# bcosm/MonteCarloOptionsPricer

Measured on AMD Instinct MI355X. Metric: Mpaths/sec at 252 steps, higher is better.
Workload: dtype f64; 1 GPU; C2: European call, GBM, 10M paths x 252 steps per GPU, fp64 matrix written; collective=none, seed=20251031

## Files before the change

### include/mcgpu_debug.h

```cpp
#ifndef MCGPU_DEBUG_H
#define MCGPU_DEBUG_H
#include "mcgpu.h"
#ifdef __cplusplus
extern "C" {
#endif

int mcg_debug_eval(mcg_ctx* ctx, int fn, const double* x, double* y, int64_t n);
int mcg_debug_lsm_hooks(mcg_ctx* ctx, long long spin_limit, int poll_delay);
int mcg_debug_lsm_date_fault(mcg_ctx* ctx, int mode, int date, int workgroup, int delay, long long spin_limit);
int mcg_debug_batch_budget(mcg_ctx* ctx, size_t bytes);
int mcg_debug_coalesce_slots(int max_slots);
int mcg_debug_coalesce_selftest(int n_threads, int calls_per_thread, int* wrong);
int mcg_debug_peer_decision(int same_process, int bus_id_resolves, int same_device, int can_access_peer);
int mcg_debug_shm_attach(const char* name, int n_ranks, int rank, double timeout_s, void** handle);
int mcg_debug_shm_barrier(void* handle);
int mcg_debug_shm_poison(void* handle);
int mcg_debug_shm_detach(void* handle);

#ifdef __cplusplus
}
#endif
#endif
```

### montecarlooptionspricer_amd/_native.py

```python
from __future__ import annotations

import ctypes as C
import os
import sys

_HERE = os.path.dirname(os.path.abspath(__file__))
_LIB = os.environ.get("MCG_LIB") or os.path.join(_HERE, "lib", "libmcgpu.so")

MCG_OK = 0
K_GBM, K_RBERGOMI, K_PAYOFF, K_LSM_SWEEP, K_LSM_SOLVE, K_TRANSPOSE, K_ASYM, K_MARTINGALE, K_BRANCHING, K_BATCH = range(10)
KERNEL_NAMES = {K_GBM: "gbm", K_RBERGOMI: "rbergomi", K_PAYOFF: "payoff", K_LSM_SWEEP: "lsm_sweep",
                K_LSM_SOLVE: "lsm_solve", K_TRANSPOSE: "transpose", K_ASYM: "asymptotic", K_MARTINGALE: "martingale", K_BRANCHING: "branching", K_BATCH: "batch_rows"}

ALLREDUCE_FN = C.CFUNCTYPE(C.c_int, C.c_void_p, C.c_void_p, C.c_int, C.c_void_p)


class Row(C.Structure):
    _fields_ = [("S0", C.c_double), ("xi", C.c_double), ("H", C.c_double), ("eta", C.c_double), ("rho", C.c_double),
                ("strike", C.c_double), ("maturity", C.c_double), ("sigma", C.c_double), ("dividend", C.c_double),
                ("n_steps", C.c_int), ("is_call", C.c_int)]


class Stats(C.Structure):
    _fields_ = [(k, C.c_int64) for k in (
# ... 36 lines not shown
    vp = C.c_void_p
    L.mcg_last_error.restype = C.c_char_p
    L.mcg_version.restype = C.c_char_p
    L.mcg_device_count.argtypes = [C.POINTER(C.c_int)]
    L.mcg_init.argtypes = [C.POINTER(vp), C.c_int]
    L.mcg_init_on_stream.argtypes = [C.POINTER(vp), C.c_int, vp]
    L.mcg_finalize.argtypes = [vp]
    L.mcg_synchronize.argtypes = [vp]
    L.mcg_trim.argtypes = [vp]
    L.mcg_set_allreduce.argtypes = [vp, ALLREDUCE_FN, vp]
    L.mcg_comm_unique_id.argtypes = [C.c_char_p]
    L.mcg_comm_init_rank.argtypes = [vp, C.c_char_p, C.c_int, C.c_int]
    L.mcg_comm_init_shm.argtypes = [vp, C.c_char_p, C.c_int, C.c_int]

    def newer(name, argtypes):
        try:
            getattr(L, name).argtypes = argtypes
        except AttributeError:
            if not os.environ.get("MCG_LIB"):
                raise

    newer("mcg_comm_shm_peer_mailbox", [vp, C.c_int, C.POINTER(C.c_int)])
    newer("mcg_debug_shm_attach", [C.c_char_p, C.c_int, C.c_int, C.c_double, C.POINTER(vp)])
    newer("mcg_debug_shm_barrier", [vp])
    newer("mcg_debug_shm_poison", [vp])
    newer("mcg_debug_shm_detach", [vp])
    newer("mcg_lsm_one_launch_reset", [vp])
    newer("mcg_debug_lsm_hooks", [vp, C.c_longlong, C.c_int])
    newer("mcg_comm_info", [vp] + [C.POINTER(C.c_int)] * 4)
    newer("mcg_timing_select", [vp, C.c_uint])
    newer("mcg_stats", [C.POINTER(Stats), C.c_int])
    newer("mcg_debug_lsm_date_fault", [vp, C.c_int, C.c_int, C.c_int, C.c_int, C.c_longlong])
    newer("mcg_debug_batch_budget", [vp, C.c_size_t])
    newer("mcg_debug_peer_decision", [C.c_int] * 4)
    newer("mcg_probe_write_ceiling", [vp, C.c_int64, C.c_int, C.c_int, C.POINTER(C.c_double), C.POINTER(C.c_double)])
    newer("mcg_generator_clock_arm", [vp, C.c_int])
    newer("mcg_generator_clock", [vp, C.POINTER(C.c_double), C.POINTER(C.c_int), C.POINTER(C.c_double), C.POINTER(C.c_double)])
    newer("mcg_row_features", [C.POINTER(C.c_double), C.c_size_t, C.POINTER(C.c_double), C.POINTER(C.c_double)])
    newer("mcg_row_build", [C.POINTER(C.c_double), C.c_size_t, C.c_double, C.c_double, C.c_double, C.c_int, C.c_double,
                            C.POINTER(Row), C.POINTER(C.c_double)])
    newer("mcg_batch_price_rows6", [vp, C.POINTER(Row), C.POINTER(C.c_double), C.c_int64, C.c_int, C.c_double, C.c_double, C.c_int,
                                    C.c_int, C.c_int, C.c_uint64, C.POINTER(C.c_double)])
    L.mcg_paths_gbm.argtypes = [vp, C.c_uint64, C.c_double, C.c_double, C.c_double, C.c_double, C.c_int,
                                C.c_uint64, C.c_int64, C.POINTER(vp)]
    L.mcg_paths_gbm_payoff.argtypes = [vp, C.c_uint64, C.c_double, C.c_double, C.c_double, C.c_double, C.c_int,
                                       C.c_uint64, C.c_int64, C.c_double, C.c_int, C.POINTER(vp)]
    L.mcg_paths_rbergomi.argtypes = [vp, C.c_uint64] + [C.c_double] * 7 + [C.c_int, C.c_uint64, C.c_int64,
                                                                          C.POINTER(vp)]
    L.mcg_paths_rbergomi_payoff.argtypes = [vp, C.c_uint64] + [C.c_double] * 7 + [C.c_int, C.c_uint64, C.c_int64,
                                                                                 C.c_double, C.c_int, C.POINTER(vp)]
    L.mcg_paths_from_host.argtypes = [vp, dp, C.c_int64, C.c_int, C.POINTER(vp)]
    L.mcg_paths_to_host.argtypes = [vp, dp]
    L.mcg_paths_to_host_step_major.argtypes = [vp, dp]
    L.mcg_paths_info.argtypes = [vp, C.POINTER(C.c_int64), C.POINTER(C.c_int), C.POINTER(C.c_int64), C.POINTER(vp)]
    L.mcg_paths_free.argtypes = [vp]
    L.mcg_price_european.argtypes = [vp, vp, C.c_double, C.c_double, C.c_double, C.c_int, dp, dp]
    L.mcg_price_lsm.argtypes = [vp, vp, C.c_double, C.c_double, C.c_double, C.c_double, C.c_int, C.c_int, dp, dp]
    L.mcg_lsm_one_launch_enabled.argtypes = [vp, C.POINTER(C.c_int)]
    L.mcg_price_asymptotic.argtypes = [vp, vp] + [C.c_double] * 4 + [C.c_int, C.c_double, C.c_double, dp]
    L.mcg_compat_asymptotic_price.argtypes = [dp, C.c_int64, C.c_int] + [C.c_double] * 4 + [C.c_int, C.c_double, C.c_double, dp]
    L.mcg_price_martingale.argtypes = [vp, vp] + [C.c_double] * 4 + [C.c_int, C.c_int, C.c_int, dp, dp, dp]
    L.mcg_compat_martingale_price.argtypes = [dp, C.c_int64, C.c_int] + [C.c_double] * 4 + [C.c_int, C.c_int, C.c_int, dp]
    ip = C.POINTER(C.c_int)
    L.mcg_price_branching.argtypes = [vp, vp] + [C.c_double] * 4 + [C.c_int, C.c_int, ip, C.c_int, C.c_uint64, dp, dp, dp]
    L.mcg_compat_branching_price.argtypes = [dp, C.c_int64, C.c_int] + [C.c_double] * 4 + [C.c_int, C.c_int, ip, C.c_int, dp]
    L.mcg_batch_price_rows.argtypes = [vp, C.POINTER(Row), C.c_int64, C.c_int, C.c_double, C.c_double, C.c_int, C.c_int,
# ... 23 lines not shown
```

### montecarlooptionspricer_amd/csrc/kernels_gbm.hip

```cpp
#include <algorithm>
#include <cstdlib>
#include <vector>

#include "devmath.hpp"
#include "fastmath.hpp"
#include "mcg_internal.hpp"

#ifndef MCG_GBM_TABLES
#define MCG_GBM_TABLES 0
#endif

namespace mcg {

struct GbmArgs {
    double* out;
    int64_t ld;
    int64_t n_paths;
    int n_steps;
    uint64_t path_begin;
    uint32_t k0, k1;
    double S0, drift, vol;
    fm::LogScale ls;
    double K;
    int is_call;
    double* partials;
    const double2* log_tab;
    unsigned long long* clk;
    unsigned clk_first, clk_shift;
};

template <bool PAYOFF, int MODE, int PPL>
__global__ __launch_bounds__(256) void k_gbm_paths(GbmArgs a) {
    constexpr bool SMALL = MODE >= 1;
    typedef double v2d __attribute__((ext_vector_type(2)));
#if MCG_GBM_TABLES == 0
    typedef fm::Tables GbmTables;
    __shared__ GbmTables tabs;
    if (MODE >= 2) fm::load_tables_scaled(&tabs, a.log_tab, a.vol * a.vol);
    else fm::load_tables(&tabs, a.log_tab);
#else
    typedef fm::NormalTables<MCG_GBM_TABLES == 1 ? 10 : 9> GbmTables;
    __shared__ GbmTables tabs;
    fm::load_normal_tables(&tabs, a.log_tab, MODE >= 2 ? a.vol * a.vol : 1.0);
#endif
    const GbmTables* tab = &tabs;
    __syncthreads();
#ifdef MCG_GBM_NO_STAMPS
    const bool stamps = false;
#else
    const bool stamps = a.clk != nullptr && (blockIdx.x & ((1u << a.clk_shift) - 1u)) == a.clk_first;
#endif
    __shared__ unsigned long long stamp0[3];
    if (threadIdx.x == 0) {
        stamp0[2] = 0;
        if (stamps && (blockIdx.x >> a.clk_shift) < (unsigned)GBM_CLK_SLOTS) {
            stamp0[2] = (unsigned long long)(a.clk + 2 * (blockIdx.x >> a.clk_shift));
            stamp0[0] = __builtin_amdgcn_s_memtime();
            stamp0[1] = __builtin_amdgcn_s_memrealtime();
        }
    }
    const int64_t i = ((int64_t)blockIdx.x * 256 + threadIdx.x) * PPL;
    const bool in_row = PPL == 1 || i < a.ld;
    double S[PPL];
#pragma unroll
    for (int p = 0; p < PPL; ++p) S[p] = a.S0;
    if (in_row) {
        double* row = a.out + (int64_t)blockIdx.x * (256 * PPL);
        const unsigned lane_bytes = threadIdx.x * (8u * PPL);
        auto store_row = [&](double* r) {
            if constexpr (PPL == 1) {
                asm volatile("global_store_dwordx2 %0, %1, %2 nt" : : "v"(lane_bytes), "v"(S[0]), "s"(r) : "memory");
            } else {
                const v2d v = {S[0], S[PPL - 1]};
                asm volatile("global_store_dwordx4 %0, %1, %2 nt\n\ts_nop 1" : : "v"(lane_bytes), "v"(v), "s"(r) : "memory");
            }
        };
        store_row(row);
        PhiloxLane lane_rng[PPL];
#pragma unroll
        for (int p = 0; p < PPL; ++p) lane_rng[p] = philox_lane_setup(a.path_begin + (uint64_t)(i + p), STREAM_PRICE, a.k1);
        auto step = [&](const double (&e)[PPL]) {
#pragma unroll
            for (int p = 0; p < PPL; ++p)
                S[p] = MODE == 3 ? fm::scaled_exp_small6(S[p], e[p]) : SMALL ? fm::scaled_exp_small(S[p], e[p]) : fm::scaled_exp(S[p], e[p]);
            row += a.ld;
            store_row(row);
        };
        auto pair_exponents = [&](uint32_t wa, uint32_t wb, double& e0, double& e1) {
            if (MODE >= 2) fm::box_muller_pair_affine_scaled(wa, wb, tab, a.ls, a.drift, e0, e1);
            else fm::box_muller_pair_affine(wa, wb, tab, a.vol, a.drift, e0, e1);
        };
        const int n_blocks = a.n_steps >> 2;
#pragma unroll 1
        for (int b = 0; b < n_blocks; ++b) {
            Philox4 w[PPL];
#pragma unroll
            for (int p = 0; p < PPL; ++p) w[p] = philox4x32_10_lane(lane_rng[p], (uint32_t)b, a.k0, a.k1);
            double e0[PPL], e1[PPL];
#pragma unroll
            for (int p = 0; p < PPL; ++p) pair_exponents(w[p].w0, w[p].w1, e0[p], e1[p]);
            step(e0);
            step(e1);
#pragma unroll
            for (int p = 0; p < PPL; ++p) pair_exponents(w[p].w2, w[p].w3, e0[p], e1[p]);
            step(e0);
            step(e1);
        }
        const int rest = a.n_steps & 3;
        if (rest) {
            Philox4 w[PPL];
#pragma unroll
            for (int p = 0; p < PPL; ++p) w[p] = philox4x32_10_lane(lane_rng[p], (uint32_t)n_blocks, a.k0, a.k1);
            double e0[PPL], e1[PPL];
#pragma unroll
            for (int p = 0; p < PPL; ++p) pair_exponents(w[p].w0, w[p].w1, e0[p], e1[p]);
            step(e0);
            if (rest >= 2) step(e1);
            if (rest == 3) {
#pragma unroll
                for (int p = 0; p < PPL; ++p) pair_exponents(w[p].w2, w[p].w3, e0[p], e1[p]);
                step(e0);
            }
        }
    }
    if (threadIdx.x == 0 && stamp0[2] != 0) {
        const unsigned long long c1 = __builtin_amdgcn_s_memtime(), r1 = __builtin_amdgcn_s_memrealtime();
        unsigned long long* dst = (unsigned long long*)stamp0[2];
        dst[0] = c1 - stamp0[0];
        dst[1] = r1 - stamp0[1];
    }
    if (PAYOFF) {
        __shared__ double red[2 * 4];
        double v[2] = {0.0, 0.0};
#pragma unroll
        for (int p = 0; p < PPL; ++p) {
            const double pay = (in_row && i + p < a.n_paths) ? payoff_of(a.is_call != 0, S[p], a.K) : 0.0;
            v[0] += pay;
            v[1] += pay * pay;
        }
        block_sum<2, 4>(v, red);
        if (threadIdx.x == 0) {
            a.partials[2 * (int64_t)blockIdx.x] = v[0];
            a.partials[2 * (int64_t)blockIdx.x + 1] = v[1];
        }
    }
}

__global__ __launch_bounds__(256) void k_payoff_sums(const double* last_row, int64_t n_paths, double K,
                                                     int is_call, double* partials) {
    __shared__ double red[2 * 4];
    double v[2] = {0.0, 0.0};
    for (int64_t i = (int64_t)blockIdx.x * 256 + threadIdx.x; i < n_paths; i += (int64_t)gridDim.x * 256) {
        const double pay = payoff_of(is_call != 0, last_row[i], K);
        v[0] += pay;
        v[1] += pay * pay;
    }
    block_sum<2, 4>(v, red);
    if (threadIdx.x == 0) {
        partials[2 * (int64_t)blockIdx.x] = v[0];
        partials[2 * (int64_t)blockIdx.x + 1] = v[1];
    }
}

constexpr int64_t FIN_CHUNK = 8192;

__device__ __forceinline__ void sum_pairs(const double* partials, int64_t n, double (&v)[2], double* red) {
    v[0] = 0.0;
    v[1] = 0.0;
    for (int64_t b = threadIdx.x; b < n; b += 1024) {
        v[0] += partials[2 * b];
        v[1] += partials[2 * b + 1];
// ... 35 lines not shown
        TimedLaunch t(ctx, MCG_K_PAYOFF);
        hipLaunchKernelGGL(k_sum_chunks, dim3((unsigned)n_chunks), dim3(1024), 0, ctx->stream, src, n, ctx->fin_chunks);
        src = ctx->fin_chunks;
        n = n_chunks;
    }
    {
        TimedLaunch t(ctx, MCG_K_PAYOFF);
        hipLaunchKernelGGL(k_finish_sums, dim3(1), dim3(1024), 0, ctx->stream, src, n, (double)n_local, d);
    }
    MCG_HIP(hipGetLastError());
    if (ctx->allreduce) {
        if (ctx->allreduce(ctx->allreduce_user, d, 3, (void*)ctx->stream) != 0)
            return fail(MCG_ERR_COMM, "all-reduce of payoff sums failed");
    }
    MCG_HIP(hipMemcpyAsync(ctx->h_scalars + SC_SUMS, d, 3 * sizeof(double), hipMemcpyDeviceToHost, ctx->stream));
    MCG_HIP(hipStreamSynchronize(ctx->stream));
    out3[0] = ctx->h_scalars[SC_SUMS];
    out3[1] = ctx->h_scalars[SC_SUMS + 1];
    out3[2] = ctx->h_scalars[SC_SUMS + 2];
    return MCG_OK;
}

template <bool PAYOFF, int PPL>
static void launch_gbm_mode(mcg_ctx* ctx, const GbmArgs& a, int mode, unsigned n_blocks) {
    const dim3 grid(n_blocks), block(256);
    if (mode == 3) hipLaunchKernelGGL((k_gbm_paths<PAYOFF, 3, PPL>), grid, block, 0, ctx->stream, a);
    else if (mode == 2) hipLaunchKernelGGL((k_gbm_paths<PAYOFF, 2, PPL>), grid, block, 0, ctx->stream, a);
    else if (mode == 1) hipLaunchKernelGGL((k_gbm_paths<PAYOFF, 1, PPL>), grid, block, 0, ctx->stream, a);
    else hipLaunchKernelGGL((k_gbm_paths<PAYOFF, 0, PPL>), grid, block, 0, ctx->stream, a);
}

static int gbm_paths_per_lane(const mcg_ctx* ctx, int64_t n_paths) {
    static const int forced = study_switch("MCG_GBM_PPL", 0);
    if (forced == 1 || forced == 2) return forced;
    return n_paths >= (int64_t)ctx->n_cus * 512 * 8 ? 2 : 1;
}

int launch_gbm(mcg_ctx* ctx, mcg_paths* P, uint64_t seed, double S0, double r, double sigma, double dt,
               bool want_payoff, double K, int is_call) {
    const int ppl = gbm_paths_per_lane(ctx, P->n_paths);
    const int64_t n_blocks = (P->n_paths + 256 * ppl - 1) / (256 * ppl);
    if (n_blocks > 0x7fffffffLL) return fail(MCG_ERR_INVALID, "n_paths too large for one launch");
    if ((P->ld & 255) != 0) return fail(MCG_ERR_INVALID, "path matrix rows must be padded to 256 columns");
    if (want_payoff) {
        int rc = ensure_cap(ctx, &ctx->partials, &ctx->partials_cap, (size_t)(2 * n_blocks));
        if (rc) return rc;
    }
    GbmArgs a;
    a.out = P->data;
    a.ld = P->ld;
    a.n_paths = P->n_paths;
    a.n_steps = P->n_steps;
    a.path_begin = P->path_begin;
    a.k0 = (uint32_t)seed;
    a.k1 = (uint32_t)(seed >> 32);
    a.S0 = S0;
    a.drift = (r - 0.5 * sigma * sigma) * dt;
    a.vol = sigma * std::sqrt(dt);
    a.K = K;
    a.is_call = is_call;
    a.partials = ctx->partials;
    a.log_tab = (const double2*)ctx->log_tab;
    a.clk = nullptr;
    a.clk_first = 0;
    a.clk_shift = 0;
    ctx->clk_slots_used = 0;
    if (ctx->clk_armed && ctx->clk_stamps && n_blocks >= 64) {
        unsigned shift = 2;
        while (((n_blocks - 1) >> shift) >= GBM_CLK_SLOTS) ++shift;
        a.clk = ctx->clk_stamps;
        a.clk_shift = shift;
        a.clk_first = (1u << shift) / 2;
        ctx->clk_slots_used = (int)(((n_blocks - 1 - a.clk_first) >> shift) + 1);
        MCG_HIP(hipMemsetAsync(ctx->clk_stamps, 0, sizeof(unsigned long long) * 2 * GBM_CLK_SLOTS, ctx->stream));
    }
    {
        TimedLaunch t(ctx, MCG_K_GBM);
        const bool small = std::fabs(a.drift) + std::fabs(a.vol) * fm::MAX_ABS_NORMAL <= fm::SMALL_EXP_BOUND;
        const double reach = std::fabs(a.drift) + std::fabs(a.vol) * fm::MAX_ABS_NORMAL;
        const int mode = !small ? 0 : !(a.vol > 1e-100) ? 1 : reach <= fm::SMALL6_EXP_BOUND ? 3 : 2;
        a.ls = fm::make_log_scale(a.vol * a.vol);
        if (want_payoff) {
            if (ppl == 2) launch_gbm_mode<true, 2>(ctx, a, mode, (unsigned)n_blocks);
            else launch_gbm_mode<true, 1>(ctx, a, mode, (unsigned)n_blocks);
        } else {
            if (ppl == 2) launch_gbm_mode<false, 2>(ctx, a, mode, (unsigned)n_blocks);
            else launch_gbm_mode<false, 1>(ctx, a, mode, (unsigned)n_blocks);
        }
    }
    MCG_HIP(hipGetLastError());
    if (want_payoff) {
        int rc = finish_sums(ctx, n_blocks, P->n_paths, P->sums);
        if (rc) return rc;
        P->has_sums = true;
        P->sums_K = K;
        P->sums_is_call = is_call;
    }
    return MCG_OK;
}

int generator_clock(mcg_ctx* ctx, double* ghz_median, int* n_stamps, double* ghz_min, double* ghz_max) {
    if (ghz_median) *ghz_median = 0.0;
    if (n_stamps) *n_stamps = 0;
    if (ghz_min) *ghz_min = 0.0;
    if (ghz_max) *ghz_max = 0.0;
    if (!ctx->clk_stamps || ctx->clk_slots_used < 1) return MCG_OK;
    unsigned long long h[2 * GBM_CLK_SLOTS];
    MCG_HIP(hipStreamSynchronize(ctx->stream));
    MCG_HIP(hipMemcpy(h, ctx->clk_stamps, sizeof h, hipMemcpyDeviceToHost));
    std::vector<double> g;
    for (int k = 0; k < ctx->clk_slots_used; ++k)
        if (h[2 * k + 1] > 100) g.push_back((double)h[2 * k] / (double)h[2 * k + 1] * 0.1);
    if (g.empty()) return MCG_OK;
    std::sort(g.begin(), g.end());
    if (ghz_median) *ghz_median = g[g.size() / 2];
    if (n_stamps) *n_stamps = (int)g.size();
    if (ghz_min) *ghz_min = g.front();
    if (ghz_max) *ghz_max = g.back();
    return MCG_OK;
}
// ... 17 lines not shown
```

### montecarlooptionspricer_amd/csrc/mcg_api.hip

```cpp
#include <algorithm>
#include <cmath>
#include <cstdlib>
#include <cstring>
#include <new>
#include <vector>

#include "fastmath_tables.hpp"
#include "mcg_internal.hpp"

namespace mcg {

static thread_local std::string g_err;
Stats g_stats;

void set_error(const char* fmt, ...) {
    char buf[512];
    va_list ap;
    va_start(ap, fmt);
    vsnprintf(buf, sizeof buf, fmt, ap);
    va_end(ap);
    g_err = buf;
}

int fail(int status, const char* fmt, ...) {
// ... 227 lines not shown
    }
    *out = ctx;
    return MCG_OK;
}

int mcg_init(mcg_ctx** out, int device) { return init_impl(out, device, false, nullptr); }

int mcg_init_on_stream(mcg_ctx** out, int device, void* stream) { return init_impl(out, device, true, stream); }

int mcg_finalize(mcg_ctx* ctx) {
    if (!ctx) return MCG_OK;
    (void)hipSetDevice(ctx->device);
    if (ctx->stream) (void)hipStreamSynchronize(ctx->stream);
    comm_release(ctx);
    shm_release(ctx);
    for (mcg_paths* P : ctx->live_paths) {
        if (P->data) (void)hipFree(P->data);
        P->data = nullptr;
        P->ctx = nullptr;
    }
    ctx->live_paths.clear();
    for (auto& b : ctx->pool) (void)hipFree(b.ptr);
    ctx->pool.clear();
    for (auto& kv : ctx->ev_live) {
        (void)hipEventDestroy(kv.second.a);
        (void)hipEventDestroy(kv.second.b);
    }
    for (auto& ev : ctx->ev_free) {
        (void)hipEventDestroy(ev.a);
        (void)hipEventDestroy(ev.b);
    }
    if (ctx->partials) (void)hipFree(ctx->partials);
    if (ctx->fin_chunks) (void)hipFree(ctx->fin_chunks);
    if (ctx->scalars) (void)hipFree(ctx->scalars);
    if (ctx->clk_stamps) (void)hipFree(ctx->clk_stamps);
    if (ctx->h_scalars) (void)hipHostFree(ctx->h_scalars);
    if (ctx->weights) (void)hipFree(ctx->weights);
    if (ctx->lsm_v) (void)hipFree(ctx->lsm_v);
    if (ctx->log_tab) (void)hipFree(ctx->log_tab);
    if (ctx->batch_fork) (void)hipEventDestroy(ctx->batch_fork);
    if (ctx->batch_join) (void)hipEventDestroy(ctx->batch_join);
    if (ctx->batch_aux) (void)hipStreamDestroy(ctx->batch_aux);
    if (ctx->owns_stream && ctx->stream) (void)hipStreamDestroy(ctx->stream);
    delete ctx;
    return MCG_OK;
}

int mcg_synchronize(mcg_ctx* ctx) {
    if (!ctx) return fail(MCG_ERR_INVALID, "ctx is NULL");
    MCG_HIP(hipStreamSynchronize(ctx->stream));
    return MCG_OK;
}

int mcg_trim(mcg_ctx* ctx) {
    if (!ctx) return fail(MCG_ERR_INVALID, "ctx is NULL");
    MCG_HIP(hipStreamSynchronize(ctx->stream));
    for (auto& b : ctx->pool) (void)hipFree(b.ptr);
    ctx->pool.clear();
    return MCG_OK;
}

int mcg_set_allreduce(mcg_ctx* ctx, mcg_allreduce_fn fn, void* user) {
    if (!ctx) return fail(MCG_ERR_INVALID, "ctx is NULL");
    shm_release(ctx);
    ctx->allreduce = fn;
    ctx->allreduce_user = user;
// ... 355 lines not shown
    return generator_clock(ctx, ghz_median, n_stamps, ghz_min, ghz_max);
}

int mcg_stats(mcg_stats_t* out, int reset) {
    if (!out && !reset) return fail(MCG_ERR_INVALID, "out is NULL");
    std::atomic<int64_t>* src[] = {&g_stats.lsm_one_launch_sweeps, &g_stats.lsm_one_launch_timeouts, &g_stats.lsm_per_date_sweeps,
                                   &g_stats.lsm_per_date_launches, &g_stats.lsm_per_date_refits, &g_stats.lsm_per_date_faults,
                                   &g_stats.shm_barrier_failures, &g_stats.peer_mailbox_enabled, &g_stats.peer_mailbox_refused,
                                   &g_stats.batch_calls, &g_stats.batch_chunks, &g_stats.batch_rows, &g_stats.batch_rows_singly,
                                   &g_stats.batch_peak_workspace_bytes, &g_stats.peer_mailbox_kept,
                                   &g_stats.coalesced_rounds, &g_stats.coalesced_calls, &g_stats.coalesced_peak_calls_per_round,
                                   &g_stats.coalesced_fallbacks, &g_stats.coalesced_round_us, &g_stats.coalesced_device_wait_us,
                                   &g_stats.coalesced_wake_us, &g_stats.coalesced_prefetched, &g_stats.coalesced_prefetch_hits};
    static_assert(sizeof(mcg_stats_t) == sizeof(src) / sizeof(src[0]) * sizeof(int64_t), "mcg_stats_t lists the counters in this order");
    int64_t* dst = reinterpret_cast<int64_t*>(out);
    for (size_t k = 0; k < sizeof(src) / sizeof(src[0]); ++k) {
        const int64_t v = reset ? src[k]->exchange(0, std::memory_order_relaxed) : src[k]->load(std::memory_order_relaxed);
        if (out) dst[k] = v;
    }
    return MCG_OK;
}

int mcg_debug_lsm_date_fault(mcg_ctx* ctx, int mode, int date, int workgroup, int delay, long long spin_limit) {
    if (!ctx) return fail(MCG_ERR_INVALID, "ctx is NULL");
    if (mode < 0 || mode > 2 || delay < 0 || delay > 100000 || spin_limit > 0xffffffffLL) return fail(MCG_ERR_INVALID, "bad hook values");
    ctx->lsm_date_hook[0] = mode;
    ctx->lsm_date_hook[1] = date;
    ctx->lsm_date_hook[2] = workgroup;
    ctx->lsm_date_hook[3] = delay;
    ctx->lsm_date_spin_limit = spin_limit;
    return MCG_OK;
}

int mcg_debug_batch_budget(mcg_ctx* ctx, size_t bytes) {
    if (!ctx) return fail(MCG_ERR_INVALID, "ctx is NULL");
    ctx->batch_budget = bytes;
    return MCG_OK;
}

int mcg_estimate_params(const double* hist, size_t n, double out5[5]) {
    if (!out5) return fail(MCG_ERR_INVALID, "out5 is NULL");
    return host_estimate_params(hist, n, out5);
}

int mcg_rbergomi_spectrum(double H, double eta, double dt, int n_steps, double* amp, double* comp, int* Mz) {
    if (n_steps < 1 || !amp || !comp) return fail(MCG_ERR_INVALID, "bad arguments");
    std::vector<double> k, c;
    int rc = host_rbergomi_spectrum(H, eta, dt, n_steps, k, c);
    if (rc) return rc;
    std::memcpy(amp, k.data(), k.size() * sizeof(double));
    std::memcpy(comp, c.data(), c.size() * sizeof(double));
    if (Mz) *Mz = (int)k.size();
    return MCG_OK;
}

int mcg_timing_enable(mcg_ctx* ctx, int on) {
    if (!ctx) return fail(MCG_ERR_INVALID, "ctx is NULL");
    ctx->timing = on != 0;
    return MCG_OK;
}

int mcg_timing_select(mcg_ctx* ctx, unsigned mask) {
    if (!ctx) return fail(MCG_ERR_INVALID, "ctx is NULL");
    ctx->timing_mask = mask;
    return MCG_OK;
}
// ... 22 lines not shown
```

### montecarlooptionspricer_amd/csrc/mcg_internal.hpp

```cpp
#pragma once
#include <hip/hip_runtime.h>
#include <stdint.h>

#include <atomic>
#include <cstdarg>
#include <cstdio>
#include <cstdlib>
#include <string>
#include <utility>
#include <vector>

#include "../../include/mcgpu.h"
#include "../../include/mcgpu_debug.h"

namespace mcg {

void set_error(const char* fmt, ...);
int fail(int status, const char* fmt, ...);

inline int study_switch(const char* name, int fallback) {
#ifdef MCG_STUDY_SWITCHES
    if (const char* e = std::getenv(name)) return std::atoi(e);
#else
    (void)name;
// ... 17 lines not shown
            return ::mcg::fail(_e == hipErrorOutOfMemory ? MCG_ERR_OOM : MCG_ERR_HIP,          \
                               "%s failed: %s (%s:%d)", #expr, hipGetErrorString(_e), __FILE__, \
                               __LINE__);                                                      \
    } while (0)

struct PoolBuf {
    void* ptr;
    size_t bytes;
};

struct EventPair {
    hipEvent_t a, b;
    int64_t launches;
};

struct ShmComm;
constexpr int SHM_MAX_RANKS = 16;
constexpr int SHM_MAX_ROUNDS = 4096;
constexpr int SHM_ROW_DOUBLES = 16;

}

struct mcg_ctx {
    int device = 0;
    hipStream_t stream = nullptr;
    bool owns_stream = false;
    int n_cus = 256;
    bool coop_launch = false;
    int coop_retry_in = 0;
    long long lsm_spin_limit = -1;
    int lsm_poll_delay = 0;
    long long lsm_date_spin_limit = -1;
    int lsm_date_hook[4] = {0, 0, 0, 0};
    size_t batch_budget = 0;
    hipStream_t batch_aux = nullptr;
    hipEvent_t batch_fork = nullptr, batch_join = nullptr;

    std::vector<mcg::PoolBuf> pool;
    std::vector<mcg_paths*> live_paths;
    double* partials = nullptr;
    size_t partials_cap = 0;
    double* fin_chunks = nullptr;
    size_t fin_chunks_cap = 0;
    double* scalars = nullptr;
    double* h_scalars = nullptr;
    double* weights = nullptr;
    size_t weights_cap = 0;
    double* lsm_v = nullptr;
    size_t lsm_v_cap = 0;
    unsigned long long* clk_stamps = nullptr;
    int clk_slots_used = 0;
    bool clk_armed = false;
    double* log_tab = nullptr;

    mcg_allreduce_fn allreduce = nullptr;
    void* allreduce_user = nullptr;
    void* rccl_comm = nullptr;
    mcg::ShmComm* shm = nullptr;
    int n_ranks = 1, rank = 0;

    bool timing = false;
    unsigned timing_mask = ~0u;
    std::vector<mcg::EventPair> ev_free;
    std::vector<std::pair<int, mcg::EventPair>> ev_live;
    double t_total[MCG_K_COUNT] = {0};
    int64_t t_count[MCG_K_COUNT] = {0};
};

struct mcg_paths {
    mcg_ctx* ctx = nullptr;
    double* data = nullptr;
    size_t bytes = 0;
    int64_t n_paths = 0;
    int n_steps = 0;
    int64_t ld = 0;
    uint64_t path_begin = 0;
// ... 82 lines not shown
```

### montecarlooptionspricer_amd/engine.py

```python
from __future__ import annotations

import ctypes as C
import weakref
from typing import Callable, Optional, Tuple

import numpy as np

from . import _native as N
from ._native import McgError, check


class _DevView:

    def __init__(self, ptr: int, count: int):
        self.__cuda_array_interface__ = {"shape": (count,), "typestr": "<f8", "data": (ptr, False),
                                         "version": 3, "strides": None}


class PathMatrix:

    def __init__(self, engine: "PathEngine", handle: C.c_void_p):
        self._engine = engine
        self._h = handle
        n_paths, n_steps, ld, ptr = C.c_int64(), C.c_int(), C.c_int64(), C.c_void_p()
# ... 212 lines not shown
        check(self._L.mcg_price_martingale(self._ctx, paths._h, r, K, maturity, dt, int(bool(is_call)), int(poly_order),
                                           int(max_iterations), C.byref(p), C.byref(lo), C.byref(up)))
        return p.value, lo.value, up.value

    def price_branching(self, paths: PathMatrix, r: float, K: float, maturity: float, dt: float, is_call: bool,
                        num_branches: int, exercise_times, seed: int) -> Tuple[float, float, float]:
        paths._alive()
        ex = np.ascontiguousarray(exercise_times, dtype=np.int32)
        p, lo, up = C.c_double(), C.c_double(), C.c_double()
        check(self._L.mcg_price_branching(self._ctx, paths._h, r, K, maturity, dt, int(bool(is_call)), int(num_branches),
                                          ex.ctypes.data_as(C.POINTER(C.c_int)), len(ex), int(seed), C.byref(p),
                                          C.byref(lo), C.byref(up)))
        return p.value, lo.value, up.value

    def batch_price_rows(self, rows, n_paths: int = 250, r: float = 0.04, dt: float = 1.0 / 252.0,
                         num_branches: int = 10, poly_order: int = 2, max_iterations: int = 5,
                         seed: int = 0, features=None) -> np.ndarray:
        arr = rows if isinstance(rows, C.Array) else make_rows(rows)
        n = len(arr)
        dp = C.POINTER(C.c_double)
        if features is None:
            out = np.zeros((n, 4), dtype=np.float64)
            check(self._L.mcg_batch_price_rows(self._ctx, arr, n, int(n_paths), r, dt, int(num_branches),
                                               int(poly_order), int(max_iterations), int(seed), out.ctypes.data_as(dp)))
            return out
        f = np.ascontiguousarray(features, dtype=np.float64)
        if f.shape != (n, 2):
            raise McgError("features must be [n_rows][2]", 1)
        out = np.zeros((n, 6), dtype=np.float64)
        check(self._L.mcg_batch_price_rows6(self._ctx, arr, f.ctypes.data_as(dp), n, int(n_paths), r, dt, int(num_branches),
                                            int(poly_order), int(max_iterations), int(seed), out.ctypes.data_as(dp)))
        return out

    def debug_batch_budget(self, nbytes: int) -> None:
        check(self._L.mcg_debug_batch_budget(self._ctx, int(nbytes)))

    def debug_lsm_date_fault(self, mode: int = 0, date: int = 0, workgroup: int = 0, delay: int = 0, spin_limit: int = -1) -> None:
        check(self._L.mcg_debug_lsm_date_fault(self._ctx, int(mode), int(date), int(workgroup), int(delay), int(spin_limit)))

    def probe_write_ceiling(self, n_paths: int = 10_000_000, n_steps: int = 252, reps: int = 5) -> Tuple[float, float]:
        g, ms = C.c_double(), C.c_double()
        check(self._L.mcg_probe_write_ceiling(self._ctx, int(n_paths), int(n_steps), int(reps), C.byref(g), C.byref(ms)))
        return g.value, ms.value

    def generator_clock_arm(self, on: bool = True) -> None:
        check(self._L.mcg_generator_clock_arm(self._ctx, 1 if on else 0))

    def generator_clock(self) -> dict:
        med, lo, hi, n = C.c_double(), C.c_double(), C.c_double(), C.c_int()
        check(self._L.mcg_generator_clock(self._ctx, C.byref(med), C.byref(n), C.byref(lo), C.byref(hi)))
        return {"GHz_median": med.value, "GHz_min": lo.value, "GHz_max": hi.value, "stamping_workgroups": n.value}

    def debug_eval(self, fn: int, x: np.ndarray) -> np.ndarray:
        x = np.ascontiguousarray(x, dtype=np.float64)
        y = np.empty((len(x), 4), dtype=np.float64)
        check(self._L.mcg_debug_eval(self._ctx, int(fn), x.ctypes.data_as(C.POINTER(C.c_double)),
                                     y.ctypes.data_as(C.POINTER(C.c_double)), len(x)))
        return y

    def timing_enable(self, on: bool = True) -> None:
        check(self._L.mcg_timing_enable(self._ctx, int(on)))

    def timing_select(self, kernels=None) -> None:
        mask = 0xFFFFFFFF if kernels is None else sum(1 << int(k) for k in kernels)
        check(self._L.mcg_timing_select(self._ctx, mask))

# ... 62 lines not shown
```

Measured before the change: 2402 Mpaths/s.

## Split final partial wave of GBM tiles into half-width workgroups

The last n_tiles mod resident-capacity tiles are launched as pairs of 256-path workgroups running one path per lane instead of one 512-path workgroup. Each pair's payoff sums are combined through a per-tile slot buffer and an atomic ticket. The aim is to spread the tail wave across more CUs and cut the idle time at the end of the launch. It adds a device workspace, atomics and a second code path, plus a debug hook to force the old schedule.

```diff
diff --git a/include/mcgpu_debug.h b/include/mcgpu_debug.h
--- a/include/mcgpu_debug.h
+++ b/include/mcgpu_debug.h
@@ -9,6 +9,7 @@
 int mcg_debug_lsm_hooks(mcg_ctx* ctx, long long spin_limit, int poll_delay);
 int mcg_debug_lsm_date_fault(mcg_ctx* ctx, int mode, int date, int workgroup, int delay, long long spin_limit);
 int mcg_debug_batch_budget(mcg_ctx* ctx, size_t bytes);
+int mcg_debug_gbm_schedule(mcg_ctx* ctx, int tile_only, int paths_per_lane);
 int mcg_debug_coalesce_slots(int max_slots);
 int mcg_debug_coalesce_selftest(int n_threads, int calls_per_thread, int* wrong);
 int mcg_debug_peer_decision(int same_process, int bus_id_resolves, int same_device, int can_access_peer);
diff --git a/montecarlooptionspricer_amd/_native.py b/montecarlooptionspricer_amd/_native.py
--- a/montecarlooptionspricer_amd/_native.py
+++ b/montecarlooptionspricer_amd/_native.py
@@ -92,6 +92,7 @@
     newer("mcg_stats", [C.POINTER(Stats), C.c_int])
     newer("mcg_debug_lsm_date_fault", [vp, C.c_int, C.c_int, C.c_int, C.c_int, C.c_longlong])
     newer("mcg_debug_batch_budget", [vp, C.c_size_t])
+    newer("mcg_debug_gbm_schedule", [vp, C.c_int, C.c_int])
     newer("mcg_debug_peer_decision", [C.c_int] * 4)
     newer("mcg_probe_write_ceiling", [vp, C.c_int64, C.c_int, C.c_int, C.POINTER(C.c_double), C.POINTER(C.c_double)])
     newer("mcg_generator_clock_arm", [vp, C.c_int])
diff --git a/montecarlooptionspricer_amd/csrc/kernels_gbm.hip b/montecarlooptionspricer_amd/csrc/kernels_gbm.hip
--- a/montecarlooptionspricer_amd/csrc/kernels_gbm.hip
+++ b/montecarlooptionspricer_amd/csrc/kernels_gbm.hip
@@ -24,15 +24,135 @@
     double K;
     int is_call;
     double* partials;
+    unsigned n_main;
+    double* tail_sums;
+    unsigned* tail_ticket;
     const double2* log_tab;
     unsigned long long* clk;
     unsigned clk_first, clk_shift;
 };
 
+template <int MODE, int PPL, typename Tab>
+__device__ __forceinline__ void gbm_lane(const GbmArgs& a, const Tab* tab, int64_t i, double* row, unsigned lane_bytes, double (&S)[PPL]) {
+    constexpr bool SMALL = MODE >= 1;
+    typedef double v2d __attribute__((ext_vector_type(2)));
+    auto store_row = [&](double* r) {
+        if constexpr (PPL == 1) {
+            asm volatile("global_store_dwordx2 %0, %1, %2 nt" : : "v"(lane_bytes), "v"(S[0]), "s"(r) : "memory");
+        } else {
+            const v2d v = {S[0], S[PPL - 1]};
+            asm volatile("global_store_dwordx4 %0, %1, %2 nt\n\ts_nop 1" : : "v"(lane_bytes), "v"(v), "s"(r) : "memory");
+        }
+    };
+    store_row(row);
+    PhiloxLane lane_rng[PPL];
+#pragma unroll
+    for (int p = 0; p < PPL; ++p) lane_rng[p] = philox_lane_setup(a.path_begin + (uint64_t)(i + p), STREAM_PRICE, a.k1);
+    auto step = [&](const double (&e)[PPL]) {
+#pragma unroll
+        for (int p = 0; p < PPL; ++p)
+            S[p] = MODE == 3 ? fm::scaled_exp_small6(S[p], e[p]) : SMALL ? fm::scaled_exp_small(S[p], e[p]) : fm::scaled_exp(S[p], e[p]);
+        row += a.ld;
+        store_row(row);
+    };
+    auto pair_exponents = [&](uint32_t wa, uint32_t wb, double& e0, double& e1) {
+        if (MODE >= 2) fm::box_muller_pair_affine_scaled(wa, wb, tab, a.ls, a.drift, e0, e1);
+        else fm::box_muller_pair_affine(wa, wb, tab, a.vol, a.drift, e0, e1);
+    };
+    const int n_blocks = a.n_steps >> 2;
+#pragma unroll 1
+    for (int b = 0; b < n_blocks; ++b) {
+        Philox4 w[PPL];
+#pragma unroll
+        for (int p = 0; p < PPL; ++p) w[p] = philox4x32_10_lane(lane_rng[p], (uint32_t)b, a.k0, a.k1);
+        double e0[PPL], e1[PPL];
+#pragma unroll
+        for (int p = 0; p < PPL; ++p) pair_exponents(w[p].w0, w[p].w1, e0[p], e1[p]);
+        step(e0);
+        step(e1);
+#pragma unroll
+        for (int p = 0; p < PPL; ++p) pair_exponents(w[p].w2, w[p].w3, e0[p], e1[p]);
+        step(e0);
+        step(e1);
+    }
+    const int rest = a.n_steps & 3;
+    if (rest) {
+        Philox4 w[PPL];
+#pragma unroll
+        for (int p = 0; p < PPL; ++p) w[p] = philox4x32_10_lane(lane_rng[p], (uint32_t)n_blocks, a.k0, a.k1);
+        double e0[PPL], e1[PPL];
+#pragma unroll
+        for (int p = 0; p < PPL; ++p) pair_exponents(w[p].w0, w[p].w1, e0[p], e1[p]);
+        step(e0);
+        if (rest >= 2) step(e1);
+        if (rest == 3) {
+#pragma unroll
+            for (int p = 0; p < PPL; ++p) pair_exponents(w[p].w2, w[p].w3, e0[p], e1[p]);
+            step(e0);
+        }
+    }
+}
+
+__device__ __forceinline__ void add_payoff(double (&v)[2], double pay) {
+    v[0] += pay;
+    v[1] += pay * pay;
+}
+
+__device__ __forceinline__ void gbm_stamp_end(const unsigned long long* stamp0) {
+    if (threadIdx.x == 0 && stamp0[2] != 0) {
+        const unsigned long long c1 = __builtin_amdgcn_s_memtime(), r1 = __builtin_amdgcn_s_memrealtime();
+        unsigned long long* dst = (unsigned long long*)stamp0[2];
+        dst[0] = c1 - stamp0[0];
+        dst[1] = r1 - stamp0[1];
+    }
+}
+
+template <bool PAYOFF, int MODE, typename Tab>
+__device__ __forceinline__ void gbm_tail_half(const GbmArgs& a, const Tab* tab, double* lds, const unsigned long long* stamp0) {
+    const unsigned u = blockIdx.x - a.n_main, t = u >> 1, h = u & 1;
+    const int64_t tile = (int64_t)a.n_main + t;
+    const int64_t c0 = tile * 512 + h * 256;
+    const int64_t i = c0 + threadIdx.x;
+    const bool in_row = c0 < a.ld;
+    double S[1] = {a.S0};
+    if (in_row) gbm_lane<MODE, 1>(a, tab, i, a.out + c0, threadIdx.x * 8u, S);
+    gbm_stamp_end(stamp0);
+    if (!PAYOFF) return;
+    const double pay = (in_row && i < a.n_paths) ? payoff_of(a.is_call != 0, S[0], a.K) : 0.0;
+    __syncthreads();
+    lds[threadIdx.x] = pay;
+    __syncthreads();
+    const int lane = threadIdx.x & 63, wave = threadIdx.x >> 6;
+    double* slot = a.tail_sums + 8 * (int64_t)t;
+    if (wave < 2) {
+        double v[2] = {0.0, 0.0};
+        add_payoff(v, lds[2 * threadIdx.x]);
+        add_payoff(v, lds[2 * threadIdx.x + 1]);
+        const WaveSums<2> r = wave_sums_folded<2>(v);
+        const double s0 = r.get(0), s1 = r.get(1);
+        if (lane == 0) {
+            __hip_atomic_store(slot + 2 * (2 * h + wave), s0, __ATOMIC_RELAXED, __HIP_MEMORY_SCOPE_AGENT);
+            __hip_atomic_store(slot + 2 * (2 * h + wave) + 1, s1, __ATOMIC_RELAXED, __HIP_MEMORY_SCOPE_AGENT);
+        }
+        __builtin_amdgcn_s_waitcnt(0);
+    }
+    __syncthreads();
+    if (threadIdx.x == 0 && __hip_atomic_fetch_add(a.tail_ticket + t, 1u, __ATOMIC_RELAXED, __HIP_MEMORY_SCOPE_AGENT) == 1u) {
+        double v[2];
+#pragma unroll
+        for (int k = 0; k < 2; ++k) {
+            double s = __hip_atomic_load(slot + k, __ATOMIC_RELAXED, __HIP_MEMORY_SCOPE_AGENT);
+            for (int w = 1; w < 4; ++w) s += __hip_atomic_load(slot + 2 * w + k, __ATOMIC_RELAXED, __HIP_MEMORY_SCOPE_AGENT);
+            v[k] = s;
+        }
+        a.partials[2 * tile] = v[0];
+        a.partials[2 * tile + 1] = v[1];
+        __hip_atomic_store(a.tail_ticket + t, 0u, __ATOMIC_RELAXED, __HIP_MEMORY_SCOPE_AGENT);
+    }
+}
+
 template <bool PAYOFF, int MODE, int PPL>
 __global__ __launch_bounds__(256) void k_gbm_paths(GbmArgs a) {
-    constexpr bool SMALL = MODE >= 1;
-    typedef double v2d __attribute__((ext_vector_type(2)));
 #if MCG_GBM_TABLES == 0
     typedef fm::Tables GbmTables;
     __shared__ GbmTables tabs;
@@ -59,84 +179,24 @@
             stamp0[1] = __builtin_amdgcn_s_memrealtime();
         }
     }
+    if (PPL == 2 && blockIdx.x >= a.n_main) {
+        gbm_tail_half<PAYOFF, MODE>(a, tab, reinterpret_cast<double*>(&tabs), stamp0);
+        return;
+    }
     const int64_t i = ((int64_t)blockIdx.x * 256 + threadIdx.x) * PPL;
     const bool in_row = PPL == 1 || i < a.ld;
     double S[PPL];
 #pragma unroll
     for (int p = 0; p < PPL; ++p) S[p] = a.S0;
-    if (in_row) {
-        double* row = a.out + (int64_t)blockIdx.x * (256 * PPL);
-        const unsigned lane_bytes = threadIdx.x * (8u * PPL);
-        auto store_row = [&](double* r) {
-            if constexpr (PPL == 1) {
-                asm volatile("global_store_dwordx2 %0, %1, %2 nt" : : "v"(lane_bytes), "v"(S[0]), "s"(r) : "memory");
-            } else {
-                const v2d v = {S[0], S[PPL - 1]};
-                asm volatile("global_store_dwordx4 %0, %1, %2 nt\n\ts_nop 1" : : "v"(lane_bytes), "v"(v), "s"(r) : "memory");
-            }
-        };
-        store_row(row);
-        PhiloxLane lane_rng[PPL];
-#pragma unroll
-        for (int p = 0; p < PPL; ++p) lane_rng[p] = philox_lane_setup(a.path_begin + (uint64_t)(i + p), STREAM_PRICE, a.k1);
-        auto step = [&](const double (&e)[PPL]) {
-#pragma unroll
-            for (int p = 0; p < PPL; ++p)
-                S[p] = MODE == 3 ? fm::scaled_exp_small6(S[p], e[p]) : SMALL ? fm::scaled_exp_small(S[p], e[p]) : fm::scaled_exp(S[p], e[p]);
-            row += a.ld;
-            store_row(row);
-        };
-        auto pair_exponents = [&](uint32_t wa, uint32_t wb, double& e0, double& e1) {
-            if (MODE >= 2) fm::box_muller_pair_affine_scaled(wa, wb, tab, a.ls, a.drift, e0, e1);
-            else fm::box_muller_pair_affine(wa, wb, tab, a.vol, a.drift, e0, e1);
-        };
-        const int n_blocks = a.n_steps >> 2;
-#pragma unroll 1
-        for (int b = 0; b < n_blocks; ++b) {
-            Philox4 w[PPL];
-#pragma unroll
-            for (int p = 0; p < PPL; ++p) w[p] = philox4x32_10_lane(lane_rng[p], (uint32_t)b, a.k0, a.k1);
-            double e0[PPL], e1[PPL];
-#pragma unroll
-            for (int p = 0; p < PPL; ++p) pair_exponents(w[p].w0, w[p].w1, e0[p], e1[p]);
-            step(e0);
-            step(e1);
-#pragma unroll
-            for (int p = 0; p < PPL; ++p) pair_exponents(w[p].w2, w[p].w3, e0[p], e1[p]);
-            step(e0);
-            step(e1);
-        }
-        const int rest = a.n_steps & 3;
-        if (rest) {
-            Philox4 w[PPL];
-#pragma unroll
-            for (int p = 0; p < PPL; ++p) w[p] = philox4x32_10_lane(lane_rng[p], (uint32_t)n_blocks, a.k0, a.k1);
-            double e0[PPL], e1[PPL];
-#pragma unroll
-            for (int p = 0; p < PPL; ++p) pair_exponents(w[p].w0, w[p].w1, e0[p], e1[p]);
-            step(e0);
-            if (rest >= 2) step(e1);
-            if (rest == 3) {
-#pragma unroll
-                for (int p = 0; p < PPL; ++p) pair_exponents(w[p].w2, w[p].w3, e0[p], e1[p]);
-                step(e0);
-            }
-        }
-    }
-    if (threadIdx.x == 0 && stamp0[2] != 0) {
-        const unsigned long long c1 = __builtin_amdgcn_s_memtime(), r1 = __builtin_amdgcn_s_memrealtime();
-        unsigned long long* dst = (unsigned long long*)stamp0[2];
-        dst[0] = c1 - stamp0[0];
-        dst[1] = r1 - stamp0[1];
-    }
+    if (in_row) gbm_lane<MODE, PPL>(a, tab, i, a.out + (int64_t)blockIdx.x * (256 * PPL), threadIdx.x * (8u * PPL), S);
+    gbm_stamp_end(stamp0);
     if (PAYOFF) {
         __shared__ double red[2 * 4];
         double v[2] = {0.0, 0.0};
 #pragma unroll
         for (int p = 0; p < PPL; ++p) {
             const double pay = (in_row && i + p < a.n_paths) ? payoff_of(a.is_call != 0, S[p], a.K) : 0.0;
-            v[0] += pay;
-            v[1] += pay * pay;
+            add_payoff(v, pay);
         }
         block_sum<2, 4>(v, red);
         if (threadIdx.x == 0) {
@@ -238,19 +298,52 @@
 
 static int gbm_paths_per_lane(const mcg_ctx* ctx, int64_t n_paths) {
     static const int forced = study_switch("MCG_GBM_PPL", 0);
+    if (ctx->gbm_ppl == 1 || ctx->gbm_ppl == 2) return ctx->gbm_ppl;
     if (forced == 1 || forced == 2) return forced;
     return n_paths >= (int64_t)ctx->n_cus * 512 * 8 ? 2 : 1;
+}
+
+static int64_t gbm_resident(const mcg_ctx* ctx) {
+    static const int per_cu = [] {
+        int n = 0;
+        if (hipOccupancyMaxActiveBlocksPerMultiprocessor(&n, (const void*)k_gbm_paths<true, 3, 2>, 256, 0) != hipSuccess || n < 1) n = 4;
+        return n;
+    }();
+    return (int64_t)per_cu * ctx->n_cus;
+}
+
+static int64_t gbm_tail_tiles(const mcg_ctx* ctx, int64_t n_tiles) {
+    static const int sched = study_switch("MCG_GBM_SCHED", 0);
+    static const int extra = study_switch("MCG_GBM_TAIL_ROUNDS", 0);
+    if (ctx->gbm_sched_tile || sched == 1) return 0;
+    const int64_t resident = gbm_resident(ctx);
+    const int64_t c = n_tiles % resident + (int64_t)extra * resident;
+    return c < n_tiles ? c : n_tiles;
 }
 
 int launch_gbm(mcg_ctx* ctx, mcg_paths* P, uint64_t seed, double S0, double r, double sigma, double dt,
                bool want_payoff, double K, int is_call) {
     const int ppl = gbm_paths_per_lane(ctx, P->n_paths);
     const int64_t n_blocks = (P->n_paths + 256 * ppl - 1) / (256 * ppl);
-    if (n_blocks > 0x7fffffffLL) return fail(MCG_ERR_INVALID, "n_paths too large for one launch");
+    const int64_t n_tail = ppl == 2 ? gbm_tail_tiles(ctx, n_blocks) : 0;
+    const int64_t n_groups = n_blocks + n_tail;
+    if (n_groups > 0x7fffffffLL) return fail(MCG_ERR_INVALID, "n_paths too large for one launch");
     if ((P->ld & 255) != 0) return fail(MCG_ERR_INVALID, "path matrix rows must be padded to 256 columns");
     if (want_payoff) {
         int rc = ensure_cap(ctx, &ctx->partials, &ctx->partials_cap, (size_t)(2 * n_blocks));
         if (rc) return rc;
+        if (n_tail > (int64_t)ctx->gbm_tail_cap) {
+            if (ctx->gbm_tail) {
+                MCG_HIP(hipStreamSynchronize(ctx->stream));
+                MCG_HIP(hipFree(ctx->gbm_tail));
+                ctx->gbm_tail = nullptr;
+                ctx->gbm_tail_cap = 0;
+            }
+            const size_t cap = (size_t)n_tail + (size_t)n_tail / 2 + 1024;
+            MCG_HIP(hipMalloc((void**)&ctx->gbm_tail, cap * (8 * sizeof(double) + sizeof(unsigned))));
+            MCG_HIP(hipMemsetAsync(ctx->gbm_tail, 0, cap * (8 * sizeof(double) + sizeof(unsigned)), ctx->stream));
+            ctx->gbm_tail_cap = cap;
+        }
     }
     GbmArgs a;
     a.out = P->data;
@@ -266,18 +359,21 @@
     a.K = K;
     a.is_call = is_call;
     a.partials = ctx->partials;
+    a.n_main = (unsigned)(n_blocks - n_tail);
+    a.tail_sums = ctx->gbm_tail;
+    a.tail_ticket = ctx->gbm_tail ? reinterpret_cast<unsigned*>(ctx->gbm_tail + 8 * ctx->gbm_tail_cap) : nullptr;
     a.log_tab = (const double2*)ctx->log_tab;
     a.clk = nullptr;
     a.clk_first = 0;
     a.clk_shift = 0;
     ctx->clk_slots_used = 0;
-    if (ctx->clk_armed && ctx->clk_stamps && n_blocks >= 64) {
+    if (ctx->clk_armed && ctx->clk_stamps && n_groups >= 64) {
         unsigned shift = 2;
-        while (((n_blocks - 1) >> shift) >= GBM_CLK_SLOTS) ++shift;
+        while (((n_groups - 1) >> shift) >= GBM_CLK_SLOTS) ++shift;
         a.clk = ctx->clk_stamps;
         a.clk_shift = shift;
         a.clk_first = (1u << shift) / 2;
-        ctx->clk_slots_used = (int)(((n_blocks - 1 - a.clk_first) >> shift) + 1);
+        ctx->clk_slots_used = (int)(((n_groups - 1 - a.clk_first) >> shift) + 1);
         MCG_HIP(hipMemsetAsync(ctx->clk_stamps, 0, sizeof(unsigned long long) * 2 * GBM_CLK_SLOTS, ctx->stream));
     }
     {
@@ -287,11 +383,11 @@
         const int mode = !small ? 0 : !(a.vol > 1e-100) ? 1 : reach <= fm::SMALL6_EXP_BOUND ? 3 : 2;
         a.ls = fm::make_log_scale(a.vol * a.vol);
         if (want_payoff) {
-            if (ppl == 2) launch_gbm_mode<true, 2>(ctx, a, mode, (unsigned)n_blocks);
-            else launch_gbm_mode<true, 1>(ctx, a, mode, (unsigned)n_blocks);
+            if (ppl == 2) launch_gbm_mode<true, 2>(ctx, a, mode, (unsigned)n_groups);
+            else launch_gbm_mode<true, 1>(ctx, a, mode, (unsigned)n_groups);
         } else {
-            if (ppl == 2) launch_gbm_mode<false, 2>(ctx, a, mode, (unsigned)n_blocks);
-            else launch_gbm_mode<false, 1>(ctx, a, mode, (unsigned)n_blocks);
+            if (ppl == 2) launch_gbm_mode<false, 2>(ctx, a, mode, (unsigned)n_groups);
+            else launch_gbm_mode<false, 1>(ctx, a, mode, (unsigned)n_groups);
         }
     }
     MCG_HIP(hipGetLastError());
diff --git a/montecarlooptionspricer_amd/csrc/mcg_api.hip b/montecarlooptionspricer_amd/csrc/mcg_api.hip
--- a/montecarlooptionspricer_amd/csrc/mcg_api.hip
+++ b/montecarlooptionspricer_amd/csrc/mcg_api.hip
@@ -283,6 +283,7 @@
     }
     if (ctx->partials) (void)hipFree(ctx->partials);
     if (ctx->fin_chunks) (void)hipFree(ctx->fin_chunks);
+    if (ctx->gbm_tail) (void)hipFree(ctx->gbm_tail);
     if (ctx->scalars) (void)hipFree(ctx->scalars);
     if (ctx->clk_stamps) (void)hipFree(ctx->clk_stamps);
     if (ctx->h_scalars) (void)hipHostFree(ctx->h_scalars);
@@ -704,6 +705,14 @@
     return MCG_OK;
 }
 
+int mcg_debug_gbm_schedule(mcg_ctx* ctx, int tile_only, int paths_per_lane) {
+    if (!ctx) return fail(MCG_ERR_INVALID, "ctx is NULL");
+    if (paths_per_lane < 0 || paths_per_lane > 2) return fail(MCG_ERR_INVALID, "paths_per_lane must be 0, 1 or 2");
+    ctx->gbm_sched_tile = tile_only != 0;
+    ctx->gbm_ppl = paths_per_lane;
+    return MCG_OK;
+}
+
 int mcg_debug_batch_budget(mcg_ctx* ctx, size_t bytes) {
     if (!ctx) return fail(MCG_ERR_INVALID, "ctx is NULL");
     ctx->batch_budget = bytes;
diff --git a/montecarlooptionspricer_amd/csrc/mcg_internal.hpp b/montecarlooptionspricer_amd/csrc/mcg_internal.hpp
--- a/montecarlooptionspricer_amd/csrc/mcg_internal.hpp
+++ b/montecarlooptionspricer_amd/csrc/mcg_internal.hpp
@@ -73,6 +73,8 @@
     int lsm_poll_delay = 0;
     long long lsm_date_spin_limit = -1;
     int lsm_date_hook[4] = {0, 0, 0, 0};
+    int gbm_ppl = 0;
+    bool gbm_sched_tile = false;
     size_t batch_budget = 0;
     hipStream_t batch_aux = nullptr;
     hipEvent_t batch_fork = nullptr, batch_join = nullptr;
@@ -83,6 +85,8 @@
     size_t partials_cap = 0;
     double* fin_chunks = nullptr;
     size_t fin_chunks_cap = 0;
+    double* gbm_tail = nullptr;
+    size_t gbm_tail_cap = 0;
     double* scalars = nullptr;
     double* h_scalars = nullptr;
     double* weights = nullptr;
diff --git a/montecarlooptionspricer_amd/engine.py b/montecarlooptionspricer_amd/engine.py
--- a/montecarlooptionspricer_amd/engine.py
+++ b/montecarlooptionspricer_amd/engine.py
@@ -268,6 +268,9 @@
                                             int(poly_order), int(max_iterations), int(seed), out.ctypes.data_as(dp)))
         return out
 
+    def debug_gbm_schedule(self, tile_only: bool = False, paths_per_lane: int = 0) -> None:
+        check(self._L.mcg_debug_gbm_schedule(self._ctx, int(bool(tile_only)), int(paths_per_lane)))
+
     def debug_batch_budget(self, nbytes: int) -> None:
         check(self._L.mcg_debug_batch_budget(self._ctx, int(nbytes)))
 
```

New measurement: 2420 Mpaths/s (median of 6 runs). Within noise of the previous version (+0.7%).
